# Quantus-Network/qp-zk-circuits

Hardware: AMD Instinct MI355X
Metric: Wormhole proofs/sec (higher is better)
Workload: dtype u64

## Files before the change

qp-zk-circuits_amd/csrc/circuit_state.hpp:

```cpp
#pragma once
#include <hip/hip_runtime.h>
#include <algorithm>
#include <vector>
#include "circuit.hpp"
#include "ctx.hpp"
#include "prover_host.hpp"
#include "prover_kernels.hpp"
#include "prover_stages.hpp"

struct WitnessPlan;
void witness_plan_free(WitnessPlan *p, qpgpu_ctx *ctx);
void witness_plan_scrub(WitnessPlan *p, hipStream_t st);

struct qpgpu_circuit {
    qpgpu_ctx *ctx = nullptr;
    CircuitPack pack;
    proof_layout::Proof layout;
    std::vector<void *> allocs;
    std::vector<std::pair<void *, size_t>> secret_allocs;
    uint32_t max_batch = 1;
    gl::u64 *d_cs_values = nullptr;
    PolyOracle cs;
    StageTables tab;
    gl::u64 *d_poseidon_fast = nullptr;
    gl::u64 *d_wires_vals = nullptr;
    uint32_t *d_salt_keys = nullptr;
    PolyOracle wires, zs, quot;
    StageWork work;
    gl::u64 *d_zs_vals = nullptr;
    gl::e2 *d_points = nullptr, *d_open = nullptr;
    FriParams fri;
    FriWork fri_work;
    Stager stage;
    bool seed_set = false;
    bool check_witness = false;
    gl::u64 blinding_seed = 0;
    WitnessPlan *wplan = nullptr;
    int witness_wide_rows = -1;

    template <class T> int alloc(T **p, size_t count, bool secret = false) {
        void *v = nullptr;
        const size_t bytes = std::max<size_t>(count * sizeof(T), 8);
        hipError_t e = ctx->track_malloc(&v, bytes, secret ? residue::CIRCUIT_WORKSPACE : residue::CIRCUIT_SETUP);
        if (e == hipErrorOutOfMemory) return ctx->fail(QPGPU_ENOMEM, "hipMalloc(circuit): out of device memory");
        if (e != hipSuccess) return ctx->hip_fail(e, "hipMalloc(circuit)");
        allocs.push_back(v);
        if (secret) secret_allocs.push_back({v, bytes});
        *p = (T *)v;
        return QPGPU_OK;
    }
};
```

qp-zk-circuits_amd/csrc/oracle_api.cpp:

```cpp
#include <hip/hip_runtime.h>
#include <algorithm>
#include <string>
#include "merkle.hpp"
#include "oracle_handle.hpp"
#include "prover_host.hpp"
#include "prover_kernels.hpp"

using gl::e2;
using gl::u64;

extern "C" void qpgpu_oracle_free(qpgpu_oracle *h) {
    if (!h) return;
    if (h->sh) { oracle_sharded_free(h); return; }
    (void)hipSetDevice(h->ctx->device);
    if (h->block) {
        (void)hipMemsetAsync(h->block, 0, h->block_words * 8, h->ctx->stream);
        (void)hipStreamSynchronize(h->ctx->stream);
        h->ctx->track_free(h->block);
    }
    delete h;
}

namespace {

int commit_impl(qpgpu_ctx *ctx, const uint64_t *const *polys, uint32_t batch, uint32_t num_polys, unsigned degree_bits, unsigned rate_bits,
                unsigned cap_height, unsigned flags, uint64_t blinding_seed, uint32_t blinding_stream, qpgpu_oracle **out) {
    if (degree_bits + rate_bits > 23 || degree_bits < 1)
        return ctx->fail(QPGPU_EINVAL, "oracle_commit: LDE sizes up to 2^23 supported");
    if (cap_height > degree_bits + rate_bits) return ctx->fail(QPGPU_EINVAL, "oracle_commit: cap_height exceeds the tree height");
    if (flags & ~7u) return ctx->fail(QPGPU_EINVAL, "oracle_commit: unknown flags");
    ctx->hasher_in_use = true;
    QP_TRY(merkle_ensure_constants(ctx));
    const bool blinding = (flags & QPGPU_ORACLE_BLINDING) != 0, from_coeffs = (flags & QPGPU_ORACLE_COEFFS) != 0;
    const u64 n = 1ull << degree_bits, lde_n = n << rate_bits;
    const unsigned L = degree_bits + rate_bits;
    const size_t B = batch;
    qpgpu_oracle *h = new qpgpu_oracle();
    h->ctx = ctx;
    PolyOracle &o = h->o;
    o.ncols = num_polys; o.log_n = degree_bits; o.rate_bits = rate_bits; o.cap_h = cap_height; o.oracle_index = blinding_stream;
    const size_t w_coeffs = (size_t)num_polys * n, w_lde = (size_t)num_polys * lde_n, w_dig = digest_words(L, cap_height),
                 w_salt = blinding ? (size_t)4 * lde_n : 0, w_eval = 2 + 2 * (size_t)num_polys;
    h->block_words = B * (w_coeffs + w_lde + w_dig + w_salt + w_eval + 4);
    void *v = nullptr;
    hipError_t e = ctx->track_malloc(&v, h->block_words * 8, residue::ORACLE);
    if (e != hipSuccess) { delete h; return ctx->hip_fail(e, "hipMalloc(oracle)"); }
    h->block = (u64 *)v;
    o.coeffs = h->block; o.lde = o.coeffs + B * w_coeffs; o.digests = o.lde + B * w_lde;
    o.salt = blinding ? o.digests + B * w_dig : nullptr;
    h->d_point = (e2 *)(o.digests + B * (w_dig + w_salt)); h->d_eval = h->d_point + B;
    h->d_key = (uint32_t *)(o.digests + B * (w_dig + w_salt + w_eval));
    o.set_batch(batch, batch == 1);
    int rc = QPGPU_OK;
    if (blinding) {
        std::vector<uint32_t> keys(8 * B);
        for (size_t b = 0; b < B && rc == QPGPU_OK; b++) {
            if (blinding_seed) salt_key_from_seed(blinding_seed + b, keys.data() + 8 * b);
            else if (salt_key_random(keys.data() + 8 * b) != QPGPU_OK) rc = ctx->fail(QPGPU_EDEVICE, "oracle_commit: the OS entropy source failed");
        }
        if (rc == QPGPU_OK) {
            e = hipMemcpyAsync(h->d_key, keys.data(), keys.size() * 4, hipMemcpyHostToDevice, ctx->stream);
            if (e == hipSuccess) e = hipStreamSynchronize(ctx->stream);
            if (e != hipSuccess) rc = ctx->hip_fail(e, "oracle_commit: key upload");
        }
        volatile uint32_t *kz = keys.data();
        for (size_t i = 0; i < keys.size(); i++) kz[i] = 0;
    }
    bool dense = true;
    for (size_t b = 0; b < B; b++) dense = dense && polys[b] == polys[0] + b * w_coeffs;
    const u64 *src = polys[0];
    if (rc == QPGPU_OK && !(flags & QPGPU_ORACLE_DEVICE_INPUT)) {
        u64 *dst = from_coeffs ? o.coeffs : o.lde;
        e = hipSuccess;
// ... 52 lines not shown
    if (!h) return QPGPU_EINVAL;
    if (coeffs) *coeffs = h->o.ps_coeffs;
    if (lde) *lde = h->o.ps_lde;
    if (digests) *digests = h->o.ps_digests;
    return QPGPU_OK;
}

int qpgpu_oracle_cap(const qpgpu_oracle *h, uint64_t *out, size_t out_words) {
    if (!h || !out || out_words < h->o.cap.size()) return QPGPU_EINVAL;
    std::memcpy(out, h->o.cap.data(), h->o.cap.size() * 8);
    return QPGPU_OK;
}

int qpgpu_oracle_eval(qpgpu_oracle *h, const uint64_t point[2], uint32_t first, uint32_t count, uint64_t *out) {
    if (!h) return QPGPU_EINVAL;
    qpgpu_ctx *ctx = h->ctx;
    QP_DEV(ctx);
    if (h->o.nb > 1) return refuse_batched(h, "oracle_eval");
    if (!point || !out || count == 0 || (size_t)first + count > h->o.ncols) return ctx->fail(QPGPU_EINVAL, "oracle_eval: bad range");
    const e2 z = gl::e2_make(gl::canon(point[0]), gl::canon(point[1]));
    QP_HIP(ctx, hipMemcpyAsync(h->d_point, &z, sizeof z, hipMemcpyHostToDevice, ctx->stream));
    QP_HIP(ctx, hipStreamSynchronize(ctx->stream));
    const u64 n = 1ull << h->o.log_n;
    QP_HIP(ctx, pk_poly_eval(h->o.coeffs + (size_t)first * n, n, count, h->d_point, 1, h->d_eval, 1, 0, 0, 0, ctx->stream));
    QP_HIP(ctx, hipMemcpyAsync(out, h->d_eval, (size_t)count * sizeof(e2), hipMemcpyDeviceToHost, ctx->stream));
    QP_HIP(ctx, hipStreamSynchronize(ctx->stream));
    return QPGPU_OK;
}

int qpgpu_oracle_read(qpgpu_oracle *h, unsigned what, uint32_t first, uint32_t count, uint64_t *out) {
    if (!h) return QPGPU_EINVAL;
    qpgpu_ctx *ctx = h->ctx;
    QP_DEV(ctx);
    if (h->o.nb > 1) return ctx->fail(QPGPU_EINVAL, "oracle_read: the oracle holds a batch of " + std::to_string(h->o.nb) + " proofs, use qpgpu_oracle_device_ptrs and qpgpu_oracle_strides");
    if (!out || count == 0 || (size_t)first + count > h->o.ncols || what > QPGPU_ORACLE_READ_LDE) return ctx->fail(QPGPU_EINVAL, "oracle_read: bad range");
    if (h->sh && what == QPGPU_ORACLE_READ_LDE) return oracle_sharded_read_lde(h, first, count, out);
    const u64 len = what == QPGPU_ORACLE_READ_LDE ? h->o.lde_n() : 1ull << h->o.log_n;
    const u64 *src = (what == QPGPU_ORACLE_READ_LDE ? h->o.lde : h->o.coeffs) + (size_t)first * len;
    QP_HIP(ctx, hipMemcpyAsync(out, src, (size_t)count * len * 8, hipMemcpyDeviceToHost, ctx->stream));
    QP_HIP(ctx, hipStreamSynchronize(ctx->stream));
    return QPGPU_OK;
}

int qpgpu_oracle_device_ptrs(const qpgpu_oracle *h, const uint64_t **d_coeffs, const uint64_t **d_lde, const uint64_t **d_digests) {
    if (!h) return QPGPU_EINVAL;
    if (h->sh) return h->ctx->fail(QPGPU_EINVAL, "oracle_device_ptrs: the oracle is sharded over " + std::to_string(h->sh->s.size()) + " contexts, use qpgpu_oracle_shard_device_ptrs");
    if (d_coeffs) *d_coeffs = h->o.coeffs;
// ... 38 lines not shown
        if (rows_out)
            for (uint32_t q = 0; q < m; q++) {
                std::memcpy(rows_out + (at + q) * width, got.data() + (size_t)q * o.ncols, (size_t)o.ncols * 8);
                if (o.salt) std::memcpy(rows_out + (at + q) * width + o.ncols, got.data() + (size_t)o.ncols * m + (size_t)q * 4, 32);
            }
        if (paths_out && plen) std::memcpy(paths_out + at * plen * 4, got.data() + (rows_out ? width * m : 0), (size_t)m * plen * 32);
    }
    return QPGPU_OK;
}

int qpgpu_oracle_eval_batch(qpgpu_oracle *h, const uint64_t *points, uint32_t first, uint32_t count, uint64_t *out) {
    if (!h) return QPGPU_EINVAL;
    qpgpu_ctx *ctx = h->ctx;
    QP_DEV(ctx);
    if (h->sh) return refuse_sharded(h, "oracle_eval_batch");
    if (!points || !out || count == 0 || (size_t)first + count > h->o.ncols) return ctx->fail(QPGPU_EINVAL, "oracle_eval_batch: bad range");
    const PolyOracle &o = h->o;
    const uint32_t nb = o.nb;
    std::vector<e2> z(nb);
    for (uint32_t b = 0; b < nb; b++) z[b] = gl::e2_make(gl::canon(points[2 * b]), gl::canon(points[2 * b + 1]));
    QP_HIP(ctx, hipMemcpyAsync(h->d_point, z.data(), nb * sizeof(e2), hipMemcpyHostToDevice, ctx->stream));
    QP_HIP(ctx, hipStreamSynchronize(ctx->stream));
    const u64 n = 1ull << o.log_n;
    QP_HIP(ctx, pk_poly_eval(o.coeffs + (size_t)first * n, n, count, h->d_point, 1, h->d_eval, nb, o.ps_coeffs, 1, count, ctx->stream));
    QP_HIP(ctx, hipMemcpyAsync(out, h->d_eval, (size_t)nb * count * sizeof(e2), hipMemcpyDeviceToHost, ctx->stream));
    QP_HIP(ctx, hipStreamSynchronize(ctx->stream));
    return QPGPU_OK;
}

int qpgpu_oracle_open_batch(qpgpu_oracle *h, const uint64_t *indices, size_t n, uint64_t *rows_out, uint64_t *paths_out) {
    if (!h) return QPGPU_EINVAL;
    qpgpu_ctx *ctx = h->ctx;
    QP_DEV(ctx);
    if (h->sh) return refuse_sharded(h, "oracle_open_batch");
    if (n == 0) return QPGPU_OK;
    if (!indices) return ctx->fail(QPGPU_EINVAL, "oracle_open_batch: indices is NULL");
    const PolyOracle &o = h->o;
    const size_t nb = o.nb;
    const u64 lde_n = o.lde_n();
    for (size_t b = 0; b < nb; b++)
        for (size_t i = 0; i < n; i++)
            if (indices[b * n + i] >= lde_n)
                return ctx->fail(QPGPU_EINVAL, "oracle_open_batch: indices[" + std::to_string(b) + "][" + std::to_string(i) + "] = " + std::to_string(indices[b * n + i]) +
                                                   " is not below 2^" + std::to_string(o.log_lde()));
    const uint32_t plen = o.log_lde() - o.cap_h;
    const size_t width = qpgpu_oracle_leaf_width(h), got_w = (rows_out ? width : 0) + (paths_out ? (size_t)plen * 4 : 0);
    if (got_w == 0) return QPGPU_OK;
// ... 65 lines not shown
```

qp-zk-circuits_amd/csrc/oracle_handle.hpp:

```cpp
#pragma once
#include <memory>
#include "oracle_shard_map.hpp"
#include "prover_host.hpp"

struct OracleShard {
    qpgpu_ctx *ctx = nullptr;
    gl::u64 *block = nullptr;
    size_t block_words = 0;
    gl::u64 *coeffs = nullptr;
    gl::u64 *lde = nullptr, *digests = nullptr, *salt = nullptr;
    uint32_t *d_key = nullptr;
};
struct OracleShards {
    qpgpu_ctx *home = nullptr;
    shard_map::Map map;
    bool blinded = false;
    std::vector<OracleShard> s;
    std::vector<gl::u64> merge;
};

struct qpgpu_oracle {
    qpgpu_ctx *ctx = nullptr;
    PolyOracle o;
    gl::u64 *block = nullptr;
    size_t block_words = 0;
    gl::e2 *d_point = nullptr, *d_eval = nullptr;
    uint32_t *d_key = nullptr;
    std::unique_ptr<OracleShards> sh;
};

void oracle_sharded_free(qpgpu_oracle *h);
int oracle_sharded_read_lde(qpgpu_oracle *h, uint32_t first, uint32_t count, uint64_t *out);
int refuse_sharded(const qpgpu_oracle *h, const char *entry);
```

qp-zk-circuits_amd/csrc/oracle_sharded.cpp:

```cpp
#include <hip/hip_runtime.h>
#include <algorithm>
#include <cstring>
#include <string>
#include "merkle.hpp"
#include "oracle_handle.hpp"
#include "prover_kernels.hpp"

using gl::u64;

namespace {
int shard_fail(qpgpu_ctx *home, uint32_t g, qpgpu_ctx *ctx, int rc) {
    if (ctx != home) home->err = "shard " + std::to_string(g) + ": " + ctx->err;
    return rc;
}
#define QP_SHARD(home, g, sctx, expr) do { int _rc = (expr); if (_rc) return shard_fail(home, g, sctx, _rc); } while (0)
#define QP_SHARD_HIP(home, g, sctx, call) do { hipError_t _e = (call); if (_e != hipSuccess) return shard_fail(home, g, sctx, (sctx)->hip_fail(_e, #call)); } while (0)

bool same_hasher(const qpgpu_ctx *a, const qpgpu_ctx *b) {
    if (a->hasher.kind != b->hasher.kind) return false;
    return a->hasher.kind != hasher::POSEIDON2 || std::memcmp(&a->hasher.p2, &b->hasher.p2, sizeof(poseidon2::Params)) == 0;
}

int commit_shards(qpgpu_oracle *h, const uint64_t *polys, unsigned flags, uint64_t blinding_seed, hipEvent_t ready) {
    qpgpu_ctx *home = h->ctx;
// ... 211 lines not shown
        for (uint32_t j = 0; j < i; j++)
            if (ctxs[i] == ctxs[j])
                return home->fail(QPGPU_EINVAL, "oracle_commit_sharded: ctxs[" + std::to_string(j) + "] and ctxs[" + std::to_string(i) + "] are the same context; every shard runs on a context of its own");
        if (!same_hasher(home, ctxs[i]))
            return home->fail(QPGPU_EINVAL, "oracle_commit_sharded: ctxs[" + std::to_string(i) + "] has another hasher than ctxs[0]");
    }
    home->hasher_in_use = true;
    QP_TRY(merkle_ensure_constants(home));

    qpgpu_oracle *h = new qpgpu_oracle();
    h->ctx = home;
    h->sh.reset(new OracleShards());
    OracleShards &sh = *h->sh;
    sh.home = home;
    sh.map.d = degree_bits; sh.map.r = rate_bits; sh.map.cap_h = cap_height; sh.map.lg = (unsigned)lg;
    sh.blinded = (flags & QPGPU_ORACLE_BLINDING) != 0;
    sh.s.resize(n_ctx);
    PolyOracle &o = h->o;
    o.ncols = num_polys; o.log_n = degree_bits; o.rate_bits = rate_bits; o.cap_h = cap_height; o.oracle_index = blinding_stream;
    o.sh = &sh; o.blinded = sh.blinded;
    o.set_batch(1, true);
    const shard_map::Map &m = sh.map;
    const u64 n = 1ull << degree_bits, Nl = m.local_leaves();
    const size_t w_coeffs = (size_t)num_polys * n, w_merge = (size_t)m.merge_digests() * 4, w_eval = 2 + 2 * (size_t)num_polys;
    const size_t w_lde = (size_t)num_polys * Nl, w_dig = digest_words(m.local_log_leaves(), m.local_cap_h()), w_salt = sh.blinded ? (size_t)4 * Nl : 0;
    int rc = QPGPU_OK;
    {
        h->block_words = w_coeffs + w_merge + w_eval;
        void *v = nullptr;
        hipError_t e = home->track_malloc(&v, h->block_words * 8, residue::ORACLE);
        if (e != hipSuccess) rc = home->hip_fail(e, "hipMalloc(oracle)");
        h->block = (u64 *)v;
        o.coeffs = h->block;
        h->d_point = (gl::e2 *)(h->block + w_coeffs + w_merge); h->d_eval = h->d_point + 1;
    }
    for (uint32_t g = 0; g < n_ctx && rc == QPGPU_OK; g++) {
        OracleShard &s = sh.s[g];
        s.ctx = ctxs[g];
        hipError_t e = hipSetDevice(s.ctx->device);
        const size_t w_copy = g ? w_coeffs : 0;
        s.block_words = w_copy + w_lde + w_dig + w_salt + 4;
        void *v = nullptr;
        if (e == hipSuccess) e = s.ctx->track_malloc(&v, s.block_words * 8, residue::ORACLE);
        if (e != hipSuccess) { rc = shard_fail(home, g, s.ctx, s.ctx->hip_fail(e, "hipMalloc(oracle shard)")); break; }
        s.block = (u64 *)v;
        s.coeffs = g ? s.block : o.coeffs;
        s.lde = s.block + w_copy; s.digests = s.lde + w_lde;
        s.salt = sh.blinded ? s.digests + w_dig : nullptr;
        s.d_key = (uint32_t *)(s.digests + w_dig + w_salt);
    }
    hipEvent_t ready = nullptr;
    if (rc == QPGPU_OK) {
        hipError_t e = hipSetDevice(home->device);
        if (e == hipSuccess) e = hipEventCreateWithFlags(&ready, hipEventDisableTiming);
        if (e != hipSuccess) rc = home->hip_fail(e, "hipEventCreate");
    }
    if (rc == QPGPU_OK) rc = commit_shards(h, polys, flags, blinding_seed, ready);
// ... 31 lines not shown
```

qp-zk-circuits_amd/csrc/prover.cpp:

```cpp
#include <hip/hip_runtime.h>
#include <algorithm>
#include <array>
#include <cstring>
#include <random>
#include <string>
#include <vector>
#include "circuit.hpp"
#include "ctx.hpp"
#include "gl64.hpp"
#include "merkle.hpp"
#include "poseidon.hpp"
#include "prover_host.hpp"
#include "circuit_state.hpp"
#include "prover_kernels.hpp"

using gl::e2;
using gl::u64;

namespace {

int alloc_batch(qpgpu_circuit *c, PolyOracle &b, uint32_t ncols, uint32_t nb, bool need_coeffs = true, uint32_t oracle_index = 0) {
    const CircuitPack &p = c->pack;
    const u64 n = p.n(), lde_n = n << p.rate_bits;
    const bool secret = oracle_index > 0;
// ... 98 lines not shown
    CK(c->alloc(&c->d_cs_values, (size_t)p.num_cs_cols() * n));
    CK(h2d_sync(ctx, c->d_cs_values, p.constants_sigmas.data(), p.constants_sigmas.size() * 8));
    CK(alloc_batch(c, c->cs, (uint32_t)p.num_cs_cols(), 1));
    CK(oracle_commit_values(ctx, c->d_cs_values, c->cs, nullptr));
    const StageAlloc take = [c](u64 **ptr, size_t count, bool secret) { return c->alloc(ptr, count, secret); };
    c->tab.cs_values = c->d_cs_values; c->tab.cs_lde = c->cs.lde;
    CK(stage_tables_build(ctx, p, take, c->tab));
    CK(c->alloc(&c->d_poseidon_fast, poseidon::FP_WORDS));
    CK(h2d_sync(ctx, c->d_poseidon_fast, poseidon::host_fast_partial(), poseidon::FP_WORDS * 8));
    unsigned qbits = 0; while ((1ull << qbits) < p.quotient_degree_factor) qbits++;
    const u64 q_n = n << qbits;
    CK(c->alloc(&c->d_wires_vals, (size_t)B * p.num_wires * n, true));
    CK(c->alloc(&c->d_salt_keys, (size_t)B * 8, true));
    CK(alloc_batch(c, c->wires, (uint32_t)p.num_wires, B, true, 1));
    CK(alloc_batch(c, c->zs, (uint32_t)p.num_zs_pp_cols(), B, true, 2));
    CK(alloc_batch(c, c->quot, (uint32_t)p.num_quotient_cols(), B, false, 3));
    CK(c->alloc(&c->quot.coeffs, (size_t)B * nch * q_n, true));
    CK(c->alloc(&c->d_zs_vals, (size_t)B * p.num_zs_pp_cols() * n, true));
    c->work.stage = &c->stage;
    CK(stage_work_alloc(p, c->tab, take, B, c->work));
    const size_t n_open = p.num_cs_cols() + p.num_wires + p.num_zs_pp_cols() + p.num_quotient_cols();
    CK(c->alloc(&c->d_points, (size_t)B * 2));
    CK(c->alloc(&c->d_open, (size_t)B * (n_open + nch), true));
    {
        c->fri.degree_bits = d; c->fri.rate_bits = (unsigned)p.rate_bits; c->fri.cap_h = (unsigned)p.cap_height;
        c->fri.pow_bits = (unsigned)p.proof_of_work_bits; c->fri.num_queries = (uint32_t)p.num_query_rounds;
        for (u64 a : p.arity_bits) c->fri.arity_bits.push_back((unsigned)a);
        const std::vector<size_t> widths(c->layout.widths, c->layout.widths + 4);
        u64 *base = nullptr;
        CK(c->alloc(&base, FriWork::words(c->fri, widths, n_open, B), true));
        c->fri_work.bind(base, c->fri, widths, n_open, B);
    }
    {
        c->stage.words = (size_t)B * (c->tab.small_words + 8 + 4 + 8) + FriWork::stage_words(c->fri, n_open, B) + 64;
        if (const char *e = getenv("QPGPU_STAGE_FALLBACK")) if (*e == '1') c->stage.words = 1;
        void *hp = nullptr;
        hipError_t e = ctx->track_host_malloc(&hp, c->stage.words * 8, residue::CIRCUIT_WORKSPACE);
        if (e != hipSuccess) return fail(ctx->hip_fail(e, "hipHostMalloc(stage)"));
        c->stage.h = (u64 *)hp;
    }
    if (const char *e = getenv("QPGPU_WITNESS_WIDE_ROWS")) if (*e == '0' || *e == '1') c->witness_wide_rows = *e - '0';
    if ((rc = ctx->reserve_read_back((size_t)B * qpgpu_proof_size(c) + (1u << 16))) != QPGPU_OK) return fail(rc);
    CK(plan_transforms(c));
    {
        const hipError_t e = hipStreamSynchronize(ctx->stream);
        if (e != hipSuccess) return fail(ctx->hip_fail(e, "circuit_load: hipStreamSynchronize"));
// ... 126 lines not shown
    ctx->prof_end();
    std::vector<e2> zetas(nb), g_zetas(nb), pts(2 * (size_t)nb);
    for (uint32_t b = 0; b < nb; b++) {
        Challenger &ch = chs[b];
        ch.observe(c->quot.cap_of(b), cap_words);
        const e2 zeta = ch.get_ext();
        {
            e2 zn = zeta;
            for (unsigned i = 0; i < d; i++) zn = gl::e2_mul(zn, zn);
            zn = gl::e2_canon(zn);
            if (zn.a == 1 && zn.b == 0) return ctx->fail(QPGPU_EINVAL, "prove: opening point is in the subgroup");
        }
        zetas[b] = zeta;
        g_zetas[b] = gl::e2_canon(gl::e2_scale(zeta, gl::root_of_unity(d)));
        pts[2 * b] = zeta; pts[2 * b + 1] = g_zetas[b];
    }

    ctx->prof_begin("prove_openings");
    const size_t n_open = ncs + NW + nzp + nq, OW = n_open + nch;
    {
        QP_TRY(c->stage.put(ctx, c->d_points, pts.data(), pts.size() * sizeof(e2)));
        const PolyOracle *bs[4] = {&c->cs, &c->wires, &c->zs, &c->quot};
        size_t off = 0;
        for (const PolyOracle *o : bs) { QP_HIP(ctx, pk_poly_eval(o->coeffs, n, o->ncols, c->d_points, 1, c->d_open + off, nb, o->ps_coeffs, 2, OW, st)); off += o->ncols; }
        QP_HIP(ctx, pk_poly_eval(c->zs.coeffs, n, nch, c->d_points + 1, 1, c->d_open + n_open, nb, c->zs.ps_coeffs, 2, OW, st));
    }
    std::vector<e2> open((size_t)nb * OW);
    QP_TRY(ctx->read_back(open.data(), c->d_open, open.size() * sizeof(e2)));
    ctx->prof_end();

    std::vector<ByteWriter> ws;
    for (uint32_t b = 0; b < nb; b++) {
        Challenger &ch = chs[b];
        const e2 *op = open.data() + (size_t)b * OW;
        ch.observe((const u64 *)op, n_open * 2);
        ch.observe((const u64 *)(op + n_open), (size_t)nch * 2);
        ws.push_back(ByteWriter{outs[b], out_cap});
        ByteWriter &w = ws.back();
        w.vec(c->wires.cap_of(b), cap_words); w.vec(c->zs.cap_of(b), cap_words); w.vec(c->quot.cap_of(b), cap_words);
        const e2 *o_cs = op, *o_w = o_cs + ncs, *o_zs = o_w + NW, *o_pp = o_zs + nch, *o_q = o_pp + (size_t)nch * npp, *o_zn = op + n_open;
        for (size_t i = 0; i < ncs; i++) w.ext(o_cs[i]);
        for (size_t i = 0; i < NW; i++) w.ext(o_w[i]);
        for (size_t i = 0; i < nch; i++) w.ext(o_zs[i]);
        for (size_t i = 0; i < nch; i++) w.ext(o_zn[i]);
        for (size_t i = 0; i < (size_t)nch * npp; i++) w.ext(o_pp[i]);
        for (size_t i = 0; i < nq; i++) w.ext(o_q[i]);
    }

// ... 64 lines not shown
```

qp-zk-circuits_amd/csrc/prover_kernels.hip:

```cpp
#include <hip/hip_runtime.h>
#include "gl64.hpp"
#include "poseidon.hpp"
#include "prover_kernels.hpp"

using gl::e2;
using gl::u32;
using gl::u64;

namespace {

__global__ void __launch_bounds__(256) pp_rows_kernel(PpArgs a) {
    const u64 i = blockIdx.x * (u64)blockDim.x + threadIdx.x;
    if (i >= a.n) return;
    const u32 k = blockIdx.y;
    { const u64 pr = blockIdx.z;
      a.wires += pr * a.ps_wires; a.betas += pr * a.ps_small; a.gammas += pr * a.ps_small; a.beta_k_is += pr * a.ps_small;
      a.qcp += pr * a.ps_qcp; a.rowprod += pr * a.ps_rowprod; }
    const u64 beta = a.betas[k], gamma = a.gammas[k];
    const u64 x = a.omega_pows[i];
    const u32 R = a.num_routed, chunk = a.chunk, nchunks = a.nchunks;
    u64 nums[16], dens[16], pref[16];
    for (u32 cc = 0; cc < nchunks; cc++) {
        u64 pn = 1, pd = 1;
        for (u32 j = cc * chunk; j < (cc + 1) * chunk && j < R; j++) {
// ... 72 lines not shown
    e2 zp[8];
    zp[0] = z;
#pragma unroll
    for (int b = 1; b < 8; b++) zp[b] = gl::e2_mul(zp[b - 1], zp[b - 1]);
    const e2 w = gl::e2_mul(zp[7], zp[7]);
    e2 acc = gl::e2_from(0);
    if (t < n) {
        const u64 terms = (n - t + T - 1) / T;
        for (u64 k = terms; k-- > 0;) acc = gl::e2_add(gl::e2_mul(acc, w), gl::e2_from(f[t + k * T]));
        e2 zt = gl::e2_from(1);
#pragma unroll
        for (int b = 0; b < 8; b++) if ((t >> b) & 1) zt = gl::e2_mul(zt, zp[b]);
        acc = gl::e2_mul(acc, zt);
    }
    part[t] = acc;
    __syncthreads();
    for (u32 off = T >> 1; off > 0; off >>= 1) {
        if (t < off) part[t] = gl::e2_add(part[t], part[t + off]);
        __syncthreads();
    }
    if (t == 0) out[(u64)blockIdx.y * gridDim.x + blockIdx.x] = gl::e2_canon(part[0]);
}

__global__ void __launch_bounds__(256) reduce_polys_kernel(const ReduceArgs a) {
    const u64 i = blockIdx.x * (u64)blockDim.x + threadIdx.x;
    if (i >= a.n) return;
    const u64 pr = blockIdx.z;
    const e2 *alpha_pows = a.alpha_pows + pr * a.ps_alpha;
    e2 acc = gl::e2_from(0);
    u32 p = 0;
    for (u32 s = 0; s < a.nsrc; s++) {
        const u64 *base = a.src[s] + pr * a.ps_src[s];
        for (u32 c = 0; c < a.ncols[s]; c++, p++) acc = gl::e2_add(acc, gl::e2_scale(alpha_pows[p], base[(u64)c * a.n + i]));
    }
    a.comp_a[pr * a.ps_comp + i] = gl::canon(acc.a);
    a.comp_b[pr * a.ps_comp + i] = gl::canon(acc.b);
}

__global__ void __launch_bounds__(1024) divide_linear_kernel(const u64 *comp_a, const u64 *comp_b, u64 n, const e2 *zs, const e2 *shifts, int mode, u64 *fin_a, u64 *fin_b,
                                                             u64 ps_comp, u64 ps_fin) {
    __shared__ e2 carry[1024];
    const u32 t = threadIdx.x, T = blockDim.x;
    const u64 pr = blockIdx.x;
    comp_a += pr * ps_comp; comp_b += pr * ps_comp; fin_a += pr * ps_fin; fin_b += pr * ps_fin;
    const e2 z = zs[pr], shift = shifts[pr];
    const u64 per = (n + T - 1) / T;
    const u64 rlo = (u64)t * per, rhi = rlo + per < n ? rlo + per : n;
    e2 acc = gl::e2_from(0);
    for (u64 r = rlo; r < rhi; r++) { const u64 i = n - 1 - r; acc = gl::e2_add(gl::e2_mul(acc, z), gl::e2_make(comp_a[i], comp_b[i])); }
    const e2 zper = gl::e2_pow(z, rhi > rlo ? rhi - rlo : 0);
    carry[t] = acc;
    __syncthreads();
    __shared__ e2 zp[1024];
    zp[t] = zper;
    __syncthreads();
    for (u32 off = 1; off < T; off <<= 1) {
        e2 c = carry[t], m = zp[t];
        if (t >= off) { c = gl::e2_add(gl::e2_mul(carry[t - off], zp[t]), carry[t]); m = gl::e2_mul(zp[t - off], zp[t]); }
        __syncthreads();
// ... 190 lines not shown
hipError_t pk_copy(void *dst, const void *src, size_t bytes, hipStream_t st) {
    if (bytes == 0) return hipSuccess;
    if ((((uintptr_t)dst | (uintptr_t)src) & 7) == 0) {
        const u64 words = bytes / 8, tail = bytes % 8;
        LAUNCH_1D(copy_words_kernel, words ? words : 1, 256, st, (u64 *)dst, (const u64 *)src, words, tail);
    } else {
        LAUNCH_1D(copy_bytes_kernel, bytes, 256, st, (unsigned char *)dst, (const unsigned char *)src, (u64)bytes);
    }
    return hipGetLastError();
}
hipError_t pk_pack_rows(const u64 *src, u64 pitch_words, u64 width_words, u64 rows, u64 *dst, hipStream_t st) {
    LAUNCH_1D(pack_rows_kernel, width_words * rows, 256, st, src, pitch_words, width_words, width_words * rows, dst);
    return hipGetLastError();
}
hipError_t pk_unpack_rows(const u64 *src, u64 pitch_words, u64 width_words, u64 rows, u64 *dst, hipStream_t st) {
    if (width_words * rows == 0) return hipSuccess;
    LAUNCH_1D(unpack_rows_kernel, width_words * rows, 256, st, src, pitch_words, width_words, width_words * rows, dst);
    return hipGetLastError();
}
hipError_t pk_scale_powers(u64 *data, u64 n, u64 ncols, const u64 *pw_lo, const u64 *pw_hi, u32 lo_bits, hipStream_t st) {
    LAUNCH_1D(scale_powers_kernel, n, 256, st, data, n, ncols, pw_lo, pw_hi, lo_bits);
    return hipGetLastError();
}
hipError_t pk_poly_eval(const u64 *coeffs, u64 n, u32 npolys, const e2 *points, u32 npoints, e2 *out, u32 batch, u64 ps_coeffs, u64 ps_points, u64 ps_out, hipStream_t st) {
    if (npolys == 0 || batch == 0) return hipSuccess;
    hipLaunchKernelGGL(poly_eval_kernel, dim3(npolys, npoints, batch), dim3(256), 0, st, coeffs, n, points, out, ps_coeffs, ps_points, ps_out);
    return hipGetLastError();
}
hipError_t pk_reduce_polys(const ReduceArgs &a, hipStream_t st) {
    LAUNCH_1D_B(reduce_polys_kernel, a.n, 256, a.batch, st, a);
    return hipGetLastError();
}
hipError_t pk_divide_linear(const u64 *comp_a, const u64 *comp_b, u64 n, const e2 *zs, const e2 *shifts, int mode, u64 *fin_a, u64 *fin_b,
                            u32 batch, u64 ps_comp, u64 ps_fin, hipStream_t st) {
    if (batch == 0) return hipSuccess;
    unsigned threads = n >= 1024 ? 1024 : (n >= 64 ? (unsigned)n : 64);
    hipLaunchKernelGGL(divide_linear_kernel, dim3(batch), dim3(threads), 0, st, comp_a, comp_b, n, zs, shifts, mode, fin_a, fin_b, ps_comp, ps_fin);
    return hipGetLastError();
}
hipError_t pk_interleave_ext(const u64 *va, const u64 *vb, u64 n, u64 *rows, u32 batch, u64 ps_vals, u64 ps_rows, hipStream_t st) {
    LAUNCH_1D_B(interleave_ext_kernel, n, 256, batch, st, va, vb, n, rows, ps_vals, ps_rows);
    return hipGetLastError();
}
hipError_t pk_fri_fold(const u64 *ca, const u64 *cb, u64 new_n, u32 arity, const e2 *betas, u64 *oa, u64 *ob, u32 batch, u64 ps_in, u64 ps_out, hipStream_t st) {
    LAUNCH_1D_B(fri_fold_kernel, new_n, 256, batch, st, ca, cb, new_n, arity, betas, oa, ob, ps_in, ps_out);
    return hipGetLastError();
}
hipError_t pk_gather_rows(const u64 *cols, u64 stride, u32 ncols, const u64 *idx, u32 nq, u64 *out, u32 batch, u64 ps_cols, u64 ps_out, hipStream_t st) {
    if (nq == 0 || batch == 0) return hipSuccess;
    hipLaunchKernelGGL(gather_rows_kernel, dim3(nq, 1, batch), dim3(128), 0, st, cols, stride, ncols, idx, nq, out, ps_cols, ps_out);
// ... 31 lines not shown
```

qp-zk-circuits_amd/csrc/prover_kernels.hpp:

```cpp
#pragma once
#include <hip/hip_runtime_api.h>
#include <stdint.h>
#include "circuit.hpp"
#include "gl64.hpp"
#include "quotient_kernels.hpp"

struct PpArgs {
    const uint64_t *wires;
    const uint64_t *sigmas;
    const uint64_t *omega_pows;
    const uint64_t *beta_k_is;
    const uint64_t *betas, *gammas;
    uint64_t *qcp;
    uint64_t *rowprod;
    uint64_t n;
    uint32_t num_routed, chunk, nchunks, nch;
    uint32_t batch;
    uint64_t ps_wires, ps_small, ps_qcp, ps_rowprod;
};

struct ReduceArgs {
    const uint64_t *src[8];
    uint64_t ps_src[8];
    uint32_t ncols[8];
    uint32_t nsrc;
    const gl::e2 *alpha_pows;
    uint64_t *comp_a, *comp_b;
    uint64_t n;
    uint32_t batch;
    uint64_t ps_alpha, ps_comp;
};

struct PowArgs {
    const uint64_t *states;
    const uint64_t *bases;
    uint64_t *results;
    uint32_t pos, pow_bits, batch;
    uint64_t count;
};

hipError_t pk_pp_rows(const PpArgs &a, hipStream_t st);
hipError_t pk_pp_scan(const uint64_t *rowprod, uint64_t *z, uint64_t n, uint32_t nch_total, hipStream_t st);
hipError_t pk_pp_finish(const PpArgs &a, const uint64_t *z, uint64_t *zs_pp, uint64_t ps_z, uint64_t ps_zs, hipStream_t st);
hipError_t pk_scale_powers(uint64_t *data, uint64_t n, uint64_t ncols, const uint64_t *pw_lo, const uint64_t *pw_hi, uint32_t lo_bits, hipStream_t st);
hipError_t pk_poly_eval(const uint64_t *coeffs, uint64_t n, uint32_t npolys, const gl::e2 *points, uint32_t npoints, gl::e2 *out,
                        uint32_t batch, uint64_t ps_coeffs, uint64_t ps_points, uint64_t ps_out, hipStream_t st);
hipError_t pk_reduce_polys(const ReduceArgs &a, hipStream_t st);
hipError_t pk_divide_linear(const uint64_t *comp_a, const uint64_t *comp_b, uint64_t n, const gl::e2 *zs, const gl::e2 *shifts, int mode,
                            uint64_t *fin_a, uint64_t *fin_b, uint32_t batch, uint64_t ps_comp, uint64_t ps_fin, hipStream_t st);
hipError_t pk_copy(void *dst, const void *src, size_t bytes, hipStream_t st);
hipError_t pk_unpack_rows(const uint64_t *src, uint64_t pitch_words, uint64_t width_words, uint64_t rows, uint64_t *dst, hipStream_t st);
hipError_t pk_pack_rows(const uint64_t *src, uint64_t pitch_words, uint64_t width_words, uint64_t rows, uint64_t *dst, hipStream_t st);
hipError_t pk_interleave_ext(const uint64_t *va, const uint64_t *vb, uint64_t n, uint64_t *rows, uint32_t batch, uint64_t ps_vals, uint64_t ps_rows, hipStream_t st);
hipError_t pk_fri_fold(const uint64_t *ca, const uint64_t *cb, uint64_t new_n, uint32_t arity, const gl::e2 *betas, uint64_t *oa, uint64_t *ob,
                       uint32_t batch, uint64_t ps_in, uint64_t ps_out, hipStream_t st);
struct HasherDev;
hipError_t pk_pow(const PowArgs &a, const HasherDev &h, hipStream_t st);
hipError_t pk_gather_rows(const uint64_t *cols, uint64_t stride, uint32_t ncols, const uint64_t *idx, uint32_t nq, uint64_t *out,
                          uint32_t batch, uint64_t ps_cols, uint64_t ps_out, hipStream_t st);
hipError_t pk_gather_paths(const uint64_t *digests, uint64_t n_leaves, uint32_t path_len, const uint64_t *idx, uint32_t shift, uint32_t nq, uint64_t *out,
                           uint32_t batch, uint64_t ps_digests, uint64_t ps_out, hipStream_t st);
hipError_t pk_gather_leaf_rows(const uint64_t *rows, uint32_t width, const uint64_t *idx, uint32_t shift, uint32_t nq, uint64_t *out,
                               uint32_t batch, uint64_t ps_rows, uint64_t ps_out, hipStream_t st);
hipError_t pk_salt(const uint32_t *keys, uint32_t oracle_index, uint64_t lde_n, uint64_t *out, uint32_t batch, hipStream_t st);
hipError_t pk_salt_slice(const uint32_t *key, uint32_t oracle_index, uint64_t first_leaf, uint64_t count, uint64_t *out, hipStream_t st);
hipError_t pk_random_felts(const uint32_t *keys, uint64_t count, uint64_t *out, uint64_t pitch, uint32_t batch, hipStream_t st);
hipError_t pk_coset_tables(uint64_t lde_n, uint32_t log_lde, uint64_t shift, const uint64_t *pw_lo, const uint64_t *pw_hi, uint32_t lo_bits, const uint64_t *zh,
                           uint32_t rate, uint64_t n_field, uint64_t *x_coset, uint64_t *l0_coset, hipStream_t st);
```

Baseline: 1598.

## Evaluate openings as dot products with precomputed point powers and lazy reduction

Opening evaluations now precompute the powers of each evaluation point once into a device table, using a two-level lo/hi power table in shared memory. A single batched dot-product kernel then evaluates all oracles' polynomials against those powers, four polynomials per block, with 192-bit accumulators and one reduction at the end. This replaces per-polynomial Horner-style evaluation launches. The reduce_polys kernel also moves to lazy 192-bit accumulation instead of a modular reduction per term. The cost is an extra device buffer of 2n extension elements per proof and one extra kernel launch.

Result: no change. 1612 (median of 6 runs) (+0.9%).

```diff
diff --git a/qp-zk-circuits_amd/csrc/circuit_state.hpp b/qp-zk-circuits_amd/csrc/circuit_state.hpp
--- a/qp-zk-circuits_amd/csrc/circuit_state.hpp
+++ b/qp-zk-circuits_amd/csrc/circuit_state.hpp
@@ -29,6 +29,7 @@
     StageWork work;
     gl::u64 *d_zs_vals = nullptr;
     gl::e2 *d_points = nullptr, *d_open = nullptr;
+    gl::e2 *d_point_pows = nullptr;
     FriParams fri;
     FriWork fri_work;
     Stager stage;
diff --git a/qp-zk-circuits_amd/csrc/oracle_api.cpp b/qp-zk-circuits_amd/csrc/oracle_api.cpp
--- a/qp-zk-circuits_amd/csrc/oracle_api.cpp
+++ b/qp-zk-circuits_amd/csrc/oracle_api.cpp
@@ -40,7 +40,8 @@
     PolyOracle &o = h->o;
     o.ncols = num_polys; o.log_n = degree_bits; o.rate_bits = rate_bits; o.cap_h = cap_height; o.oracle_index = blinding_stream;
     const size_t w_coeffs = (size_t)num_polys * n, w_lde = (size_t)num_polys * lde_n, w_dig = digest_words(L, cap_height),
-                 w_salt = blinding ? (size_t)4 * lde_n : 0, w_eval = 2 + 2 * (size_t)num_polys;
+                 w_salt = blinding ? (size_t)4 * lde_n : 0, w_pow = n % 256 ? 0 : 2 * (size_t)n,
+                 w_eval = 2 + 2 * (size_t)num_polys + w_pow;
     h->block_words = B * (w_coeffs + w_lde + w_dig + w_salt + w_eval + 4);
     void *v = nullptr;
     hipError_t e = ctx->track_malloc(&v, h->block_words * 8, residue::ORACLE);
@@ -49,6 +50,7 @@
     o.coeffs = h->block; o.lde = o.coeffs + B * w_coeffs; o.digests = o.lde + B * w_lde;
     o.salt = blinding ? o.digests + B * w_dig : nullptr;
     h->d_point = (e2 *)(o.digests + B * (w_dig + w_salt)); h->d_eval = h->d_point + B;
+    if (w_pow) h->d_pow = h->d_eval + B * num_polys;
     h->d_key = (uint32_t *)(o.digests + B * (w_dig + w_salt + w_eval));
     o.set_batch(batch, batch == 1);
     int rc = QPGPU_OK;
@@ -147,7 +149,8 @@
     QP_HIP(ctx, hipMemcpyAsync(h->d_point, &z, sizeof z, hipMemcpyHostToDevice, ctx->stream));
     QP_HIP(ctx, hipStreamSynchronize(ctx->stream));
     const u64 n = 1ull << h->o.log_n;
-    QP_HIP(ctx, pk_poly_eval(h->o.coeffs + (size_t)first * n, n, count, h->d_point, 1, h->d_eval, 1, 0, 0, 0, ctx->stream));
+    QP_HIP(ctx, pk_point_powers(h->d_point, 1, n, h->d_pow, ctx->stream));
+    QP_HIP(ctx, pk_poly_eval(h->o.coeffs + (size_t)first * n, n, count, h->d_point, 1, h->d_eval, 1, 0, 0, 0, ctx->stream, h->d_pow, n));
     QP_HIP(ctx, hipMemcpyAsync(out, h->d_eval, (size_t)count * sizeof(e2), hipMemcpyDeviceToHost, ctx->stream));
     QP_HIP(ctx, hipStreamSynchronize(ctx->stream));
     return QPGPU_OK;
@@ -232,7 +235,8 @@
     QP_HIP(ctx, hipMemcpyAsync(h->d_point, z.data(), nb * sizeof(e2), hipMemcpyHostToDevice, ctx->stream));
     QP_HIP(ctx, hipStreamSynchronize(ctx->stream));
     const u64 n = 1ull << o.log_n;
-    QP_HIP(ctx, pk_poly_eval(o.coeffs + (size_t)first * n, n, count, h->d_point, 1, h->d_eval, nb, o.ps_coeffs, 1, count, ctx->stream));
+    QP_HIP(ctx, pk_point_powers(h->d_point, nb, n, h->d_pow, ctx->stream));
+    QP_HIP(ctx, pk_poly_eval(o.coeffs + (size_t)first * n, n, count, h->d_point, 1, h->d_eval, nb, o.ps_coeffs, 1, count, ctx->stream, h->d_pow, n));
     QP_HIP(ctx, hipMemcpyAsync(out, h->d_eval, (size_t)nb * count * sizeof(e2), hipMemcpyDeviceToHost, ctx->stream));
     QP_HIP(ctx, hipStreamSynchronize(ctx->stream));
     return QPGPU_OK;
diff --git a/qp-zk-circuits_amd/csrc/oracle_handle.hpp b/qp-zk-circuits_amd/csrc/oracle_handle.hpp
--- a/qp-zk-circuits_amd/csrc/oracle_handle.hpp
+++ b/qp-zk-circuits_amd/csrc/oracle_handle.hpp
@@ -25,6 +25,7 @@
     gl::u64 *block = nullptr;
     size_t block_words = 0;
     gl::e2 *d_point = nullptr, *d_eval = nullptr;
+    gl::e2 *d_pow = nullptr;
     uint32_t *d_key = nullptr;
     std::unique_ptr<OracleShards> sh;
 };
diff --git a/qp-zk-circuits_amd/csrc/oracle_sharded.cpp b/qp-zk-circuits_amd/csrc/oracle_sharded.cpp
--- a/qp-zk-circuits_amd/csrc/oracle_sharded.cpp
+++ b/qp-zk-circuits_amd/csrc/oracle_sharded.cpp
@@ -257,7 +257,8 @@
     o.set_batch(1, true);
     const shard_map::Map &m = sh.map;
     const u64 n = 1ull << degree_bits, Nl = m.local_leaves();
-    const size_t w_coeffs = (size_t)num_polys * n, w_merge = (size_t)m.merge_digests() * 4, w_eval = 2 + 2 * (size_t)num_polys;
+    const size_t w_coeffs = (size_t)num_polys * n, w_merge = (size_t)m.merge_digests() * 4, w_pow = n % 256 ? 0 : 2 * (size_t)n,
+                 w_eval = 2 + 2 * (size_t)num_polys + w_pow;
     const size_t w_lde = (size_t)num_polys * Nl, w_dig = digest_words(m.local_log_leaves(), m.local_cap_h()), w_salt = sh.blinded ? (size_t)4 * Nl : 0;
     int rc = QPGPU_OK;
     {
@@ -268,6 +269,7 @@
         h->block = (u64 *)v;
         o.coeffs = h->block;
         h->d_point = (gl::e2 *)(h->block + w_coeffs + w_merge); h->d_eval = h->d_point + 1;
+        if (w_pow) h->d_pow = h->d_eval + num_polys;
     }
     for (uint32_t g = 0; g < n_ctx && rc == QPGPU_OK; g++) {
         OracleShard &s = sh.s[g];
diff --git a/qp-zk-circuits_amd/csrc/prover.cpp b/qp-zk-circuits_amd/csrc/prover.cpp
--- a/qp-zk-circuits_amd/csrc/prover.cpp
+++ b/qp-zk-circuits_amd/csrc/prover.cpp
@@ -144,6 +144,7 @@
     const size_t n_open = p.num_cs_cols() + p.num_wires + p.num_zs_pp_cols() + p.num_quotient_cols();
     CK(c->alloc(&c->d_points, (size_t)B * 2));
     CK(c->alloc(&c->d_open, (size_t)B * (n_open + nch), true));
+    if (n % 256 == 0) CK(c->alloc(&c->d_point_pows, (size_t)B * 2 * n, true));
     {
         c->fri.degree_bits = d; c->fri.rate_bits = (unsigned)p.rate_bits; c->fri.cap_h = (unsigned)p.cap_height;
         c->fri.pow_bits = (unsigned)p.proof_of_work_bits; c->fri.num_queries = (uint32_t)p.num_query_rounds;
@@ -316,8 +317,20 @@
         QP_TRY(c->stage.put(ctx, c->d_points, pts.data(), pts.size() * sizeof(e2)));
         const PolyOracle *bs[4] = {&c->cs, &c->wires, &c->zs, &c->quot};
         size_t off = 0;
-        for (const PolyOracle *o : bs) { QP_HIP(ctx, pk_poly_eval(o->coeffs, n, o->ncols, c->d_points, 1, c->d_open + off, nb, o->ps_coeffs, 2, OW, st)); off += o->ncols; }
-        QP_HIP(ctx, pk_poly_eval(c->zs.coeffs, n, nch, c->d_points + 1, 1, c->d_open + n_open, nb, c->zs.ps_coeffs, 2, OW, st));
+        if (c->d_point_pows) {
+            QP_HIP(ctx, pk_point_powers(c->d_points, 2 * nb, n, c->d_point_pows, st));
+            PolyEvalArgs ea = {};
+            for (const PolyOracle *o : bs) {
+                ea.src[ea.nsrc] = o->coeffs; ea.ps_src[ea.nsrc] = o->ps_coeffs; ea.ncols[ea.nsrc] = o->ncols; ea.point[ea.nsrc] = 0; ea.out_off[ea.nsrc++] = (uint32_t)off;
+                off += o->ncols;
+            }
+            ea.src[4] = c->zs.coeffs; ea.ps_src[4] = c->zs.ps_coeffs; ea.ncols[4] = nch; ea.point[4] = 1; ea.out_off[4] = (uint32_t)n_open;
+            ea.nsrc = 5; ea.batch = nb; ea.n = n; ea.pows = c->d_point_pows; ea.ps_pows = 2 * n; ea.out = c->d_open; ea.ps_out = OW;
+            QP_HIP(ctx, pk_poly_eval_dot(ea, st));
+        } else {
+            for (const PolyOracle *o : bs) { QP_HIP(ctx, pk_poly_eval(o->coeffs, n, o->ncols, c->d_points, 1, c->d_open + off, nb, o->ps_coeffs, 2, OW, st)); off += o->ncols; }
+            QP_HIP(ctx, pk_poly_eval(c->zs.coeffs, n, nch, c->d_points + 1, 1, c->d_open + n_open, nb, c->zs.ps_coeffs, 2, OW, st));
+        }
     }
     std::vector<e2> open((size_t)nb * OW);
     QP_TRY(ctx->read_back(open.data(), c->d_open, open.size() * sizeof(e2)));
diff --git a/qp-zk-circuits_amd/csrc/prover_kernels.hip b/qp-zk-circuits_amd/csrc/prover_kernels.hip
--- a/qp-zk-circuits_amd/csrc/prover_kernels.hip
+++ b/qp-zk-circuits_amd/csrc/prover_kernels.hip
@@ -118,19 +118,91 @@
     if (t == 0) out[(u64)blockIdx.y * gridDim.x + blockIdx.x] = gl::e2_canon(part[0]);
 }
 
+__global__ void __launch_bounds__(256) point_powers_kernel(const e2 *points, u64 n, e2 *pows) {
+    __shared__ e2 lo[257], hi[256];
+    const u32 t = threadIdx.x;
+    if (t == 0) { lo[0] = gl::e2_from(1); lo[1] = points[blockIdx.y]; hi[0] = gl::e2_from(1); }
+    __syncthreads();
+    for (u32 m = 1; m <= 128; m <<= 1) {
+        if (t >= 1 && t <= m) lo[m + t] = gl::e2_mul(lo[m], lo[t]);
+        __syncthreads();
+    }
+    if (t == 0) hi[1] = lo[256];
+    __syncthreads();
+    for (u32 m = 1; m <= 128; m <<= 1) {
+        if (t >= 1 && t <= m && m + t < 256) hi[m + t] = gl::e2_mul(hi[m], hi[t]);
+        __syncthreads();
+    }
+    const u64 first = (u64)blockIdx.x << 16;
+    const u32 nhi = (u32)((n - first) / 256 < 256 ? (n - first) / 256 : 256);
+    const e2 base = gl::e2_pow(lo[256], (u64)blockIdx.x << 8), mine = lo[t];
+    e2 *dst = pows + (u64)blockIdx.y * n + first + t;
+    for (u32 j = 0; j < nhi; j++) {
+        e2 v = gl::e2_mul(hi[j], mine);
+        if (blockIdx.x) v = gl::e2_mul(v, base);
+        dst[(u64)j * 256] = gl::e2_canon(v);
+    }
+}
+
+constexpr int POLY_EVAL_TILE = 4;
+__global__ void __launch_bounds__(256) poly_eval_dot_kernel(const PolyEvalArgs a) {
+    constexpr int PT = POLY_EVAL_TILE;
+    __shared__ u64 part[4][2 * PT];
+    const u32 t = threadIdx.x;
+    const u64 pr = blockIdx.y, n = a.n;
+    u32 tile = blockIdx.x, s = 0;
+    while (s + 1 < a.nsrc && tile >= (a.ncols[s] + PT - 1) / PT) { tile -= (a.ncols[s] + PT - 1) / PT; s++; }
+    const u32 npolys = a.ncols[s], p0 = tile * PT;
+    const e2 *pw = a.pows + pr * a.ps_pows + (u64)a.point[s] * n + t;
+    const u64 *coeffs = a.src[s] + pr * a.ps_src[s];
+    const u64 *f[PT];
+#pragma unroll
+    for (int p = 0; p < PT; p++) f[p] = coeffs + (u64)(p0 + p < npolys ? p0 + p : npolys - 1) * n + t;
+    gl::Acc192 acc_a[PT], acc_b[PT];
+#pragma unroll
+    for (int p = 0; p < PT; p++) { acc_a[p] = gl::acc_zero(); acc_b[p] = gl::acc_zero(); }
+    for (u64 i = 0; i < n; i += 256) {
+        const e2 w = pw[i];
+        u64 c[PT];
+#pragma unroll
+        for (int p = 0; p < PT; p++) c[p] = f[p][i];
+#pragma unroll
+        for (int p = 0; p < PT; p++) { gl::acc_mul(acc_a[p], c[p], w.a); gl::acc_mul(acc_b[p], c[p], w.b); }
+    }
+#pragma unroll
+    for (int p = 0; p < PT; p++) {
+        u64 va = gl::acc_reduce(acc_a[p]), vb = gl::acc_reduce(acc_b[p]);
+#pragma unroll
+        for (int off = 32; off > 0; off >>= 1) { va = gl::add(va, __shfl_xor(va, off)); vb = gl::add(vb, __shfl_xor(vb, off)); }
+        if ((t & 63) == 0) { part[t >> 6][2 * p] = va; part[t >> 6][2 * p + 1] = vb; }
+    }
+    __syncthreads();
+    if (t < PT && p0 + t < npolys) {
+        e2 r = gl::e2_make(part[0][2 * t], part[0][2 * t + 1]);
+#pragma unroll
+        for (int w = 1; w < 4; w++) r = gl::e2_add(r, gl::e2_make(part[w][2 * t], part[w][2 * t + 1]));
+        a.out[pr * a.ps_out + a.out_off[s] + p0 + t] = gl::e2_canon(r);
+    }
+}
+
 __global__ void __launch_bounds__(256) reduce_polys_kernel(const ReduceArgs a) {
     const u64 i = blockIdx.x * (u64)blockDim.x + threadIdx.x;
     if (i >= a.n) return;
     const u64 pr = blockIdx.z;
     const e2 *alpha_pows = a.alpha_pows + pr * a.ps_alpha;
-    e2 acc = gl::e2_from(0);
+    gl::Acc192 acc_a = gl::acc_zero(), acc_b = gl::acc_zero();
     u32 p = 0;
     for (u32 s = 0; s < a.nsrc; s++) {
         const u64 *base = a.src[s] + pr * a.ps_src[s];
-        for (u32 c = 0; c < a.ncols[s]; c++, p++) acc = gl::e2_add(acc, gl::e2_scale(alpha_pows[p], base[(u64)c * a.n + i]));
-    }
-    a.comp_a[pr * a.ps_comp + i] = gl::canon(acc.a);
-    a.comp_b[pr * a.ps_comp + i] = gl::canon(acc.b);
+        for (u32 c = 0; c < a.ncols[s]; c++, p++) {
+            const e2 al = alpha_pows[p];
+            const u64 f = base[(u64)c * a.n + i];
+            gl::acc_mul(acc_a, al.a, f);
+            gl::acc_mul(acc_b, al.b, f);
+        }
+    }
+    a.comp_a[pr * a.ps_comp + i] = gl::canon(gl::acc_reduce(acc_a));
+    a.comp_b[pr * a.ps_comp + i] = gl::canon(gl::acc_reduce(acc_b));
 }
 
 __global__ void __launch_bounds__(1024) divide_linear_kernel(const u64 *comp_a, const u64 *comp_b, u64 n, const e2 *zs, const e2 *shifts, int mode, u64 *fin_a, u64 *fin_b,
@@ -367,10 +439,29 @@
     LAUNCH_1D(scale_powers_kernel, n, 256, st, data, n, ncols, pw_lo, pw_hi, lo_bits);
     return hipGetLastError();
 }
-hipError_t pk_poly_eval(const u64 *coeffs, u64 n, u32 npolys, const e2 *points, u32 npoints, e2 *out, u32 batch, u64 ps_coeffs, u64 ps_points, u64 ps_out, hipStream_t st) {
+hipError_t pk_point_powers(const e2 *points, u32 count, u64 n, e2 *pows, hipStream_t st) {
+    if (count == 0 || n == 0 || n % 256) return hipSuccess;
+    hipLaunchKernelGGL(point_powers_kernel, dim3((unsigned)((n + 65535) >> 16), count), dim3(256), 0, st, points, n, pows);
+    return hipGetLastError();
+}
+hipError_t pk_poly_eval_dot(const PolyEvalArgs &a, hipStream_t st) {
+    u32 tiles = 0;
+    for (u32 s = 0; s < a.nsrc; s++) tiles += (a.ncols[s] + POLY_EVAL_TILE - 1) / POLY_EVAL_TILE;
+    if (tiles == 0 || a.batch == 0) return hipSuccess;
+    hipLaunchKernelGGL(poly_eval_dot_kernel, dim3(tiles, a.batch), dim3(256), 0, st, a);
+    return hipGetLastError();
+}
+hipError_t pk_poly_eval(const u64 *coeffs, u64 n, u32 npolys, const e2 *points, u32 npoints, e2 *out, u32 batch, u64 ps_coeffs, u64 ps_points, u64 ps_out, hipStream_t st,
+                        const e2 *pows, u64 ps_pows) {
     if (npolys == 0 || batch == 0) return hipSuccess;
-    hipLaunchKernelGGL(poly_eval_kernel, dim3(npolys, npoints, batch), dim3(256), 0, st, coeffs, n, points, out, ps_coeffs, ps_points, ps_out);
-    return hipGetLastError();
+    if (!pows || n % 256 || npoints > 8) {
+        hipLaunchKernelGGL(poly_eval_kernel, dim3(npolys, npoints, batch), dim3(256), 0, st, coeffs, n, points, out, ps_coeffs, ps_points, ps_out);
+        return hipGetLastError();
+    }
+    PolyEvalArgs a = {};
+    for (u32 y = 0; y < npoints; y++) { a.src[y] = coeffs; a.ps_src[y] = ps_coeffs; a.ncols[y] = npolys; a.point[y] = y; a.out_off[y] = y * npolys; }
+    a.nsrc = npoints; a.n = n; a.batch = batch; a.pows = pows; a.ps_pows = ps_pows; a.out = out; a.ps_out = ps_out;
+    return pk_poly_eval_dot(a, st);
 }
 hipError_t pk_reduce_polys(const ReduceArgs &a, hipStream_t st) {
     LAUNCH_1D_B(reduce_polys_kernel, a.n, 256, a.batch, st, a);
diff --git a/qp-zk-circuits_amd/csrc/prover_kernels.hpp b/qp-zk-circuits_amd/csrc/prover_kernels.hpp
--- a/qp-zk-circuits_amd/csrc/prover_kernels.hpp
+++ b/qp-zk-circuits_amd/csrc/prover_kernels.hpp
@@ -31,6 +31,17 @@
     uint64_t ps_alpha, ps_comp;
 };
 
+struct PolyEvalArgs {
+    const uint64_t *src[8];
+    uint64_t ps_src[8];
+    uint32_t ncols[8], point[8], out_off[8];
+    uint32_t nsrc, batch;
+    uint64_t n;
+    const gl::e2 *pows;
+    gl::e2 *out;
+    uint64_t ps_pows, ps_out;
+};
+
 struct PowArgs {
     const uint64_t *states;
     const uint64_t *bases;
@@ -43,8 +54,11 @@
 hipError_t pk_pp_scan(const uint64_t *rowprod, uint64_t *z, uint64_t n, uint32_t nch_total, hipStream_t st);
 hipError_t pk_pp_finish(const PpArgs &a, const uint64_t *z, uint64_t *zs_pp, uint64_t ps_z, uint64_t ps_zs, hipStream_t st);
 hipError_t pk_scale_powers(uint64_t *data, uint64_t n, uint64_t ncols, const uint64_t *pw_lo, const uint64_t *pw_hi, uint32_t lo_bits, hipStream_t st);
+hipError_t pk_point_powers(const gl::e2 *points, uint32_t count, uint64_t n, gl::e2 *pows, hipStream_t st);
+hipError_t pk_poly_eval_dot(const PolyEvalArgs &a, hipStream_t st);
 hipError_t pk_poly_eval(const uint64_t *coeffs, uint64_t n, uint32_t npolys, const gl::e2 *points, uint32_t npoints, gl::e2 *out,
-                        uint32_t batch, uint64_t ps_coeffs, uint64_t ps_points, uint64_t ps_out, hipStream_t st);
+                        uint32_t batch, uint64_t ps_coeffs, uint64_t ps_points, uint64_t ps_out, hipStream_t st,
+                        const gl::e2 *pows = nullptr, uint64_t ps_pows = 0);
 hipError_t pk_reduce_polys(const ReduceArgs &a, hipStream_t st);
 hipError_t pk_divide_linear(const uint64_t *comp_a, const uint64_t *comp_b, uint64_t n, const gl::e2 *zs, const gl::e2 *shifts, int mode,
                             uint64_t *fin_a, uint64_t *fin_b, uint32_t batch, uint64_t ps_comp, uint64_t ps_fin, hipStream_t st);
```
